# matheusfalcaopinto/triple-hybrid-rag

Hardware: AMD Instinct MI355X
Metric: queries/sec (fused top-10) (higher is better)
Workload: dtype f16 MFMA shortlist scan (f32 accumulate) + f64 rescoring of the f32 rows

## Files before the change

### triple-hybrid-rag_amd/csrc/dense.hip

```cpp
#include <stdlib.h>

#include "dense_common.hpp"

namespace thr {

constexpr double QREG_AIM_1M = 1448.0;
constexpr int QREG_KS = 32;
struct DenseKnobs {
    bool forced_q;
    int shape;
    bool forced32;
    double aim_1m;
    int ks;
};
static const DenseKnobs& dense_knobs() {
    static const DenseKnobs knobs = [] {
        DenseKnobs K;
        const char* e = getenv("THR_DENSE_F16");
        K.forced_q = e && e[0] == 'q';
        e = getenv("THR_DENSE_MFMA");
        K.shape = (e && atoi(e) == 32) ? 32 : 16;
        e = getenv("THR_DENSE_QW");
        K.forced32 = e && atoi(e) == 32;
        e = getenv("THR_DENSE_AIM");
        K.aim_1m = (e && atof(e) >= 64.0) ? atof(e) : QREG_AIM_1M;
        e = getenv("THR_DENSE_KS");
        K.ks = (e && atoi(e) >= 4 && atoi(e) <= 64) ? atoi(e) : QREG_KS;
        return K;
    }();
    return knobs;
}

bool qreg_staggered(int dim) { return !dense_knobs().forced_q && dim <= 768; }
int qreg_waves(int dim) { return qreg_staggered(dim) ? 8 : 4; }
int qreg_shape(int) { return dense_knobs().shape; }
int qreg_qw(int dim) {
    return (dim == 1024 && !qreg_staggered(dim) && qreg_shape(dim) == 16 && !dense_knobs().forced32) ? 48 : 32;
}
int qreg_max_queries(int dim) {
    const int qt = qreg_qw(dim) * qreg_waves(dim);
    const int64_t m = (int64_t)UINT32_MAX / ((int64_t)CAND_CAP * (int64_t)sizeof(Cand));
    return (int)(m / qt * qt);
}


static thread_local int f16_selected = THR_DENSE_F16_BY_DIM;
static bool f16_tuned_dim(int dim) { return dim == 512 || dim == 768 || dim == 1024; }
static bool f16_dim_ok(int dim, bool packed) { return f16_tuned_dim(dim) || (!packed && anydim_ok(dim)); }
static bool f16_anydim(int dim, bool packed) {
    return !packed && anydim_ok(dim) && (!f16_tuned_dim(dim) || f16_selected == THR_DENSE_F16_ANYDIM);
}

static DensePlan make_plan(void* ws, int64_t n_docs, int n_queries, int kprime, int kind, int dim,
                           bool packed) {
    DensePlan p;
    p.kind = kind;
    p.packed = kind == KIND_F16 && packed;
    p.anydim = kind == KIND_F16 && f16_anydim(dim, p.packed);
    p.nq = (kind == KIND_F16 && !p.packed && !p.anydim) ? f16_pick_nq(dim) : 1;
    p.row_bits = (kind == KIND_F16 && !p.packed) ? ROW_BITS_F16 : ROW_BITS;
    p.qtile = p.packed ? qreg_qw(dim) * qreg_waves(dim)
              : p.anydim ? anydim_qt(dim)
              : kind == KIND_F16 ? 32 * p.nq : MF_QT;
    p.ntiles = (n_queries + p.qtile - 1) / p.qtile;
    p.qpad = p.ntiles * p.qtile;
    const int64_t groups = (n_docs + MF_ROWS - 1) / MF_ROWS;
    p.sampled = n_docs > CAND_CAP / 2;
    const int ks_cap = p.packed ? dense_knobs().ks : 64;
    p.ksample = kprime < ks_cap ? kprime : ks_cap;
    double aim = (p.packed ? dense_knobs().aim_1m : 4096.0) * sqrt((double)n_docs / 1.0e6);
    const double aim_lo = 8.0 * kprime < 4096.0 ? 8.0 * kprime : 4096.0;
    aim = aim < aim_lo ? aim_lo : aim > 4096.0 ? 4096.0 : aim;
    int64_t target = (int64_t)((double)n_docs * (double)p.ksample / aim);
    if (target > SAMPLE_MAX) target = SAMPLE_MAX;
    if (target < 4 * (int64_t)p.ksample) target = 4 * (int64_t)p.ksample;
    int64_t sg = (target + MF_ROWS - 1) / MF_ROWS;
    if (sg > groups) sg = groups;
    p.sample_stride = sg > 0 ? groups / sg : 1;
    if (p.sample_stride < 1) p.sample_stride = 1;
    p.sample_groups = p.sampled ? sg : 0;
    p.sample_docs = p.sample_groups * MF_ROWS;
    p.groups = groups;
    p.tile_cap = p.packed ? 1 : p.qtile * (CAND_CAP / 2);
    const size_t qpad = (size_t)p.qpad;
    Arena A{(char*)ws};
    p.tau = A.take<float>(qpad);
    p.qerr = A.take<float>(qpad);
    if (kind != KIND_F16) p.qerr = nullptr;
    p.cnt = A.take<int>(qpad * (p.packed ? QREG_MAX_SEG : 1));
    p.tcnt = A.take<int>(p.ntiles);
    p.cand = A.take<Cand>(qpad * CAND_CAP);
    p.tlist = A.take<Cand>((size_t)p.ntiles * p.tile_cap);
    p.sample = A.take<float>(p.packed ? qpad * (size_t)QREG_MAX_SEG * SAMPLE_TOP : qpad * (size_t)p.sample_docs);
    p.qfrag = A.take<_Float16>(p.packed ? qpad * (size_t)dim : 0);
    p.sel_rows = A.take<int32_t>(qpad * SEL_BIG_BAND);
    p.sel_meta = A.take<int32_t>(4 * qpad);
    p.total = A.total;
    return p;
}

dim3 scan_grid(int ntiles, int64_t n_row_tiles, int waves, bool* shared_rows, int blocks_per_cu,
               int m_cap) {
    const int cus = num_cus() * blocks_per_cu;
    int64_t m_max = n_row_tiles / (8 * (int64_t)waves);
    if (m_max < 1) m_max = 1;
    if (m_max > m_cap) m_max = m_cap;
    int best_m = 1;
    double best_eff = 0.0;
    for (int m = 1; m <= (int)m_max; ++m) {
        const int64_t g = 8 * (int64_t)m * ntiles;
        const int64_t rounds = (g + cus - 1) / cus;
        const double eff = (double)g / (double)(rounds * cus);
        if (eff > best_eff + 1e-9) {
            best_eff = eff;
            best_m = m;
        }
    }
    *shared_rows = ntiles > 1;
    return dim3((unsigned)(8 * best_m * ntiles), 1u);
}

bool scan_nt(bool shared_rows) { return !shared_rows; }


template <int MODE>
static int launch_scan(const DensePlan& P, const DenseIndex& X, const DenseBatch& B, int* nseg = nullptr) {
    constexpr bool all = MODE == MODE_ALL;
    const int64_t units = all ? P.sample_groups : P.groups, stride = all ? P.sample_stride : 1;
    const float* tau = all ? nullptr : P.tau;
    float* smp = all ? P.sample : nullptr;
    const int64_t ld = all ? P.sample_docs : 0;
    if (P.packed)
        return launch_scan_f16q<MODE>(X.dim, X.docs16, P.qfrag, P.ntiles, units, stride, tau,
                                      all ? nullptr : P.cnt, all ? nullptr : P.cand, smp, B.st,
                                      nseg, X.doc_coll, B.query_coll, B.n_queries);
    const int32_t* doc_coll = all ? nullptr : X.doc_coll;
    const int32_t* query_coll = all ? nullptr : B.query_coll;
    int* tcnt = all ? nullptr : P.tcnt;
    Cand* tlist = all ? nullptr : P.tlist;
    const int tile_cap = all ? 0 : P.tile_cap;
    if (P.anydim)
        return launch_scan_anydim<MODE>(X.dim, X.docs, X.inv_norm, X.n_docs, B.queries, B.n_queries, P.ntiles,
                                        units, stride, tau, tcnt, tlist, tile_cap, smp, ld, B.st, doc_coll,
                                        query_coll);
    if (P.kind == KIND_F16)
        return launch_scan_f16<MODE>(X.dim, P.nq, X.docs, X.inv_norm, X.n_docs, B.queries, B.n_queries,
                                     P.ntiles, units, stride, tau, tcnt, tlist, tile_cap, smp, ld, B.st,
                                     doc_coll, query_coll);
    return launch_scan_mfma<MODE>(X.dim, X.docs, X.inv_norm, X.n_docs, B.queries, B.n_queries, P.ntiles,
                                  units, stride, tau, tcnt, tlist, tile_cap, smp, ld, B.st, doc_coll,
                                  query_coll);
}

static int dense_pipeline(const DensePlan& P, const DenseIndex& X, const DenseBatch& B,
                          const DensePhase& S) {
    int rc, nseg = 0, sample_nseg = 0;
    if (S.phase != PIPE_FINISH) {
        if (!P.packed) {
            hipError_t e = hipMemsetAsync(P.cnt, 0, (char*)P.cand - (char*)P.cnt, B.st);
            if (e != hipSuccess) return (int)e;
        }
        if (P.packed && (rc = launch_pack_queries(X.dim, B.queries, B.n_queries, P.qpad, P.qfrag, P.qerr, B.st)))
            return rc;
        if (P.sampled && (rc = launch_scan<MODE_ALL>(P, X, B, &sample_nseg))) return rc;
        if ((rc = launch_threshold(P, X, B, P.packed ? sample_nseg : 0))) return rc;
        if ((rc = launch_scan<MODE_FILTER>(P, X, B, &nseg))) return rc;
        if (!P.packed && (rc = launch_bucket(P, B.st))) return rc;
    } else if (P.packed) {
        if ((rc = launch_scan_f16q<MODE_FILTER, true>(X.dim, X.docs16, P.qfrag, P.ntiles, P.groups, 1,
                                                      nullptr, nullptr, nullptr, nullptr, B.st, &nseg)))
            return rc;
    }
    if ((rc = launch_band(P, X, B, S, nseg))) return rc;
    if (S.phase == PIPE_SHORTLIST) return THR_OK;
    return launch_rescore(P, X, B);
}

}

using namespace thr;

extern "C" size_t thr_dense_workspace_bytes(int64_t n_docs, int dim, int n_queries, int kprime) {
    if (n_docs <= 0 || n_queries <= 0) return 0;
    return make_plan(nullptr, n_docs, n_queries, kprime, KIND_F32, dim, false).total;
}

static int dense_args_ok(const void* docs, const void* dnorm, const void* inv_norm,
                         const void* queries, const void* a, const void* b, const void* c,
                         const void* d, const void* ws, int64_t n_docs, int n_queries, int k,
                         int kprime) {
    THR_RETURN_IF(!docs || !dnorm || !inv_norm || !queries || !a || !b || !c || !d || !ws,
                  THR_ERR_INVALID);
    THR_RETURN_IF(n_docs <= 0 || n_queries <= 0 || k <= 0 || kprime < k ||
                      kprime > THR_DENSE_MAX_K,
                  THR_ERR_INVALID);
    return THR_OK;
}

extern "C" int thr_dense_topk(const float* docs, const double* dnorm, const float* inv_norm,
                              int64_t n_docs, int dim, int64_t id_base, const float* queries,
                              int n_queries, int k, int kprime, const int32_t* doc_coll,
                              const int32_t* query_coll, double* out_scores,
                              int64_t* out_ids, int32_t* out_counts, uint32_t* out_flags,
                              void* workspace, size_t workspace_bytes, thr_stream_t stream) {
    clear_status();
    int rc = dense_args_ok(docs, dnorm, inv_norm, queries, out_scores, out_ids, out_counts,
                           out_flags, workspace, n_docs, n_queries, k, kprime);
    if (rc) return rc;
    THR_RETURN_IF((query_coll != nullptr) != (doc_coll != nullptr), THR_ERR_INVALID);
    THR_RETURN_IF(dim <= 0 || dim % CHUNK != 0 || dim / CHUNK > 4, THR_ERR_UNSUPPORTED);
    THR_RETURN_IF(n_docs >= (int64_t)1 << ROW_BITS, THR_ERR_UNSUPPORTED);
    const DensePlan P = make_plan(workspace, n_docs, n_queries, kprime, KIND_F32, dim, false);
    THR_RETURN_IF(workspace_bytes < P.total, THR_ERR_WORKSPACE);
    const DenseIndex X{docs, inv_norm, n_docs, dim, dnorm, id_base, doc_coll};
    const DenseBatch B{queries, n_queries, k, kprime, query_coll, (hipStream_t)stream,
                       out_scores, out_ids, out_counts, out_flags};
    return dense_pipeline(P, X, B, DensePhase{});
}

extern "C" size_t thr_dense_f16_workspace_bytes(int64_t n_docs, int dim, int n_queries,
                                                int kprime) {
    if (n_docs <= 0 || n_queries <= 0) return 0;
    const size_t a = make_plan(nullptr, n_docs, n_queries, kprime, KIND_F16, dim, false).total;
    if (anydim_ok(dim) && !f16_tuned_dim(dim)) return a;
    const size_t b = make_plan(nullptr, n_docs, n_queries, kprime, KIND_F16, dim, true).total;
    return a > b ? a : b;
}

extern "C" int thr_dense_f16_select(int flavour) {
    const int before = f16_selected;
    if (!f16_tiles_agree()) return before;
    if (flavour == THR_DENSE_F16_BY_DIM || flavour == THR_DENSE_F16_ANYDIM) f16_selected = flavour;
    return before;
}

extern "C" int thr_dense_f16_max_queries(int dim, int packed) {
    if (!f16_dim_ok(dim, packed != 0)) return 0;
    return packed ? qreg_max_queries(dim) : INT32_MAX;
}

extern "C" int thr_dense_f16_query_tile(int dim, int packed, int n_queries) {
    if (!f16_dim_ok(dim, packed != 0)) return 0;
    (void)n_queries;
    if (f16_anydim(dim, packed != 0)) return anydim_qt(dim);
    return packed ? qreg_qw(dim) * qreg_waves(dim) : 32 * f16_pick_nq(dim);
// ... 159 lines not shown
```

### triple-hybrid-rag_amd/csrc/dense_common.hpp

```cpp
#pragma once
#include <type_traits>

#include "thr_common.hpp"

namespace thr {

constexpr int CHUNK = 256;
constexpr int MODE_ALL = 0, MODE_FILTER = 1;
constexpr int CAND_CAP = 16384;
constexpr int SAMPLE_MAX = 1 << 20;
constexpr int WBUF = 256;
constexpr int ROW_BITS = 27;
constexpr uint32_t ROW_MASK = (1u << ROW_BITS) - 1;
constexpr int ROW_BITS_F16 = 25;
constexpr int SEL_BIG_BAND = 1024;
constexpr int QREG_MAX_SEG = 1024;
constexpr int SAMPLE_TOP = 4;
constexpr int CS_BINS = 4096;

struct Cand {
    float score;
    uint32_t doc;
};

// ... 42 lines not shown
    const half4 a = __builtin_convertvector(lo, half4), b = __builtin_convertvector(hi, half4);
    half8 v = {a[0], a[1], a[2], a[3], b[0], b[1], b[2], b[3]};
    return __builtin_bit_cast(f32x4, v);
}

inline size_t f16_lds_bytes(int dim, int nq) {
    return sizeof(_Float16) * 32 * nq * (size_t)dim +
           (sizeof(Cand) * WBUF + sizeof(float4) * MF2_STAGE_F4) * H_WAVES;
}
inline int f16_pick_nq(int dim) { return f16_lds_bytes(dim, 2) <= 160 * 1024 ? 2 : 1; }

inline bool anydim_ok(int dim) {
    return dim >= THR_DENSE_ANYDIM_STEP && dim <= THR_DENSE_ANYDIM_MAX && dim % THR_DENSE_ANYDIM_STEP == 0;
}
inline int anydim_qt(int dim) { return dim <= 768 ? 64 : dim <= 1536 ? 32 : 16; }
inline size_t anydim_lds_bytes(int dim) {
    return sizeof(_Float16) * (size_t)anydim_qt(dim) * (size_t)dim + sizeof(Cand) * WBUF * H_WAVES;
}

inline bool f16_tiles_agree() {
    for (int dim : {512, 768, 1024})
        if (anydim_qt(dim) != 32 * f16_pick_nq(dim)) return false;
    return true;
}

inline double scan_eps(int dim) {
    const double u = 5.9604644775390625e-08;
    return ((double)dim + 16.0) * u;
}

constexpr int KIND_F32 = 0, KIND_F16 = 1;
struct DensePlan {
    int kind;
    bool anydim;
    bool packed;
    int nq, qtile, ntiles, qpad, row_bits, ksample, tile_cap;
    bool sampled;
    int64_t groups, sample_groups, sample_stride, sample_docs;
    float* tau;
    float* qerr;
    int* cnt;
    int* tcnt;
    Cand *cand, *tlist;
    float* sample;
    _Float16* qfrag;
    int32_t *sel_rows, *sel_meta;
    size_t total;
};
struct DenseIndex {
    const float *docs, *inv_norm;
    int64_t n_docs;
    int dim;
    const double* dnorm = nullptr;
    int64_t id_base = 0;
    const int32_t* doc_coll = nullptr;
    const _Float16* docs16 = nullptr;
    double doc_rel_err = 0.0;
};
struct DenseBatch {
    const float* queries;
    int n_queries, k, kprime;
    const int32_t* query_coll;
    hipStream_t st;
    double* out_scores = nullptr;
    int64_t* out_ids = nullptr;
    int32_t* out_counts = nullptr;
    uint32_t* out_flags = nullptr;
};
enum { PIPE_ALL = 0, PIPE_SHORTLIST = 1, PIPE_FINISH = 2 };
struct DensePhase {
    int phase = PIPE_ALL;
    float* top_lb = nullptr;
    int top_m = 0;
    const float* gfloor = nullptr;
    const float* lb_all = nullptr;
    int n_shards = 0;
};

bool qreg_staggered(int dim);
int qreg_waves(int dim);
int qreg_shape(int dim);
int qreg_qw(int dim);
int qreg_max_queries(int dim);
dim3 scan_grid(int ntiles, int64_t n_row_tiles, int waves, bool* shared_rows, int blocks_per_cu = 1,
               int m_cap = 64);
bool scan_nt(bool shared_rows);

template <int MODE>
int launch_scan_mfma(int dim, const float* docs, const float* inv_norm, int64_t n_docs,
                     const float* queries, int n_queries, int ntiles, int64_t n_row_tiles,
                     int64_t tile_stride, const float* tau, int* tile_cnt, Cand* tile_list,
                     int tile_cap, float* sample, int64_t sample_ld, hipStream_t st,
                     const int32_t* doc_coll = nullptr, const int32_t* query_coll = nullptr);
template <int MODE>
int launch_scan_f16(int dim, int nq, const float* rows32, const float* inv_norm, int64_t n_docs,
                    const float* queries, int n_queries, int ntiles, int64_t n_row_tiles,
                    int64_t tile_stride, const float* tau, int* tile_cnt, Cand* tile_list,
                    int tile_cap, float* sample, int64_t sample_ld, hipStream_t st,
                    const int32_t* doc_coll = nullptr, const int32_t* query_coll = nullptr);
template <int MODE>
int launch_scan_anydim(int dim, const float* rows32, const float* inv_norm, int64_t n_docs,
                       const float* queries, int n_queries, int ntiles, int64_t n_row_tiles,
                       int64_t tile_stride, const float* tau, int* tile_cnt, Cand* tile_list,
                       int tile_cap, float* sample, int64_t sample_ld, hipStream_t st,
                       const int32_t* doc_coll = nullptr, const int32_t* query_coll = nullptr);
template <int MODE, bool PROF = false>
int launch_scan_f16q(int dim, const _Float16* rows16, const _Float16* qfrag, int n_qtiles,
                     int64_t n_row_tiles, int64_t tile_stride, const float* tau, int* seg_cnt,
                     Cand* cand, float* sample, hipStream_t st,
                     int* nseg_out = nullptr, const int32_t* doc_coll = nullptr,
                     const int32_t* query_coll = nullptr, int n_queries = 1 << 30,
                     unsigned long long* stamps = nullptr, int* n_blocks = nullptr);
int launch_pack_queries(int dim, const float* queries, int n_queries, int qpad, _Float16* qfrag,
                        float* qerr, hipStream_t st);
int launch_quantize_f16(const float* docs, int64_t n_docs, int dim, _Float16* docs16,
                        unsigned int* max_rel_err, hipStream_t st);
int launch_threshold(const DensePlan& P, const DenseIndex& X, const DenseBatch& B, int sample_nseg);
int launch_bucket(const DensePlan& P, hipStream_t st);
int launch_band(const DensePlan& P, const DenseIndex& X, const DenseBatch& B, const DensePhase& S, int nseg);
int launch_rescore(const DensePlan& P, const DenseIndex& X, const DenseBatch& B);
int launch_merge_scoped(const double* slab_s, const int64_t* slab_id, int n_queries, int n_slabs, int k,
                        int64_t id_base, const int32_t* query_scope, int n_scopes, double* out_scores,
                        int64_t* out_ids, int32_t* out_counts, uint32_t* out_flags, hipStream_t st);

}
```

### triple-hybrid-rag_amd/csrc/dense_scan_f16q.hip

```cpp
#include "dense_scan_f16q.hpp"

namespace thr {

template <int MODE, bool PROF>
int launch_scan_f16q(int dim, const _Float16* rows16, const _Float16* qfrag, int n_qtiles,
                            int64_t n_row_tiles, int64_t tile_stride, const float* tau, int* seg_cnt,
                            Cand* cand, float* sample, hipStream_t st,
                            int* nseg_out, const int32_t* doc_coll,
                            const int32_t* query_coll, int n_queries,
                            unsigned long long* stamps, int* n_blocks) {
    bool shared_rows = false;
    const bool stag = qreg_staggered(dim);
    const dim3 grid = scan_grid(n_qtiles, n_row_tiles, 1, &shared_rows, (!stag && dim <= 768) ? 2 : 1, 32);
    const int shape = qreg_shape(dim);
    const int nseg = (shape == 16 ? 4 : 2) * (int)(grid.x / n_qtiles);
    if (nseg_out) *nseg_out = nseg;
    if (n_blocks) *n_blocks = (int)grid.x;
    if (PROF && !stamps) return THR_OK;
#define THR_QS_LAUNCH(DIM, SHAPE)                                                                 \
    return launch_lds(dense_scan_f16qs<DIM, MODE, SHAPE>, grid, dim3(QS_NW * 64),                 \
                      QStag<DIM>::LDS_BYTES, st, (const f32x4*)rows16, (const f32x4*)qfrag,       \
                      n_qtiles, n_row_tiles, tile_stride, tau, seg_cnt, cand, CAND_CAP / nseg,    \
                      sample, doc_coll, query_coll, n_queries);
    if (stag) {
        if (dim == 512 && shape == 32) THR_QS_LAUNCH(512, 32)
        if (dim == 512) THR_QS_LAUNCH(512, 16)
        if (shape == 32) THR_QS_LAUNCH(768, 32)
        THR_QS_LAUNCH(768, 16)
    }
#undef THR_QS_LAUNCH
#define THR_Q_LAUNCH(DIM, SHAPE)                                                                  \
    return launch_lds(dense_scan_f16q<DIM, MODE, PROF, SHAPE>, grid, dim3(Q_NW * 64),             \
                      QScan<DIM>::LDS_BYTES, st, (const f32x4*)rows16, (const f32x4*)qfrag,       \
                      n_qtiles, n_row_tiles, tile_stride, tau, seg_cnt, cand, CAND_CAP / nseg,    \
                      sample, doc_coll, query_coll, n_queries, stamps);
    switch (dim) {
        case 512: if (shape == 16) THR_Q_LAUNCH(512, 16) THR_Q_LAUNCH(512, 32)
        case 768: if (shape == 16) THR_Q_LAUNCH(768, 16) THR_Q_LAUNCH(768, 32)
        case 1024:
            if (shape == 16 && qreg_qw(dim) == 48) THR_Q_LAUNCH(1024, 48)
            if (shape == 16) THR_Q_LAUNCH(1024, 16)
            THR_Q_LAUNCH(1024, 32)
        default: return THR_ERR_UNSUPPORTED;
    }
#undef THR_Q_LAUNCH
}

int launch_pack_queries(int dim, const float* queries, int n_queries, int qpad,
                               _Float16* qfrag, float* qerr, hipStream_t st) {
    const dim3 grid((unsigned)(qpad / 32));
    const bool s16 = qreg_shape(dim) == 16;
#define THR_PACK(DIM, SHAPE) \
    hipLaunchKernelGGL((pack_queries_f16<DIM, SHAPE>), grid, dim3(256), 0, st, queries, n_queries, (f32x4*)qfrag, qerr)
    switch (dim) {
        case 512: if (s16) THR_PACK(512, 16); else THR_PACK(512, 32); break;
        case 768: if (s16) THR_PACK(768, 16); else THR_PACK(768, 32); break;
        case 1024: if (s16) THR_PACK(1024, 16); else THR_PACK(1024, 32); break;
        default: return THR_ERR_UNSUPPORTED;
    }
#undef THR_PACK
    return launch_status();
}

int launch_quantize_f16(const float* docs, int64_t n_docs, int dim, _Float16* docs16,
                        unsigned int* max_rel_err, hipStream_t st) {
    if (docs16) {
        THR_RETURN_IF(dim % 16 != 0, THR_ERR_UNSUPPORTED);
        const int64_t n_pad = (n_docs + 31) / 32 * 32;
        hipLaunchKernelGGL(quantize_f16_norm, dim3((unsigned)((n_pad + 3) / 4)), dim3(256), 0, st,
                           docs, n_docs, dim, qreg_shape(dim), docs16, max_rel_err);
        return launch_status();
    }
    hipLaunchKernelGGL(measure_f16_error, dim3((unsigned)((n_docs + 3) / 4)), dim3(256), 0, st, docs,
                       n_docs, dim, max_rel_err);
    return launch_status();
}

#define THR_INSTANTIATE(MODE, PROF)                                                                    \
    template int launch_scan_f16q<MODE, PROF>(int, const _Float16*, const _Float16*, int, int64_t, int64_t, \
                                              const float*, int*, Cand*, float*, hipStream_t, int*, \
                                              const int32_t*, const int32_t*, int, unsigned long long*, int*);
THR_INSTANTIATE(MODE_ALL, false)
THR_INSTANTIATE(MODE_FILTER, false)
THR_INSTANTIATE(MODE_FILTER, true)
#undef THR_INSTANTIATE

}
```

### triple-hybrid-rag_amd/csrc/dense_scan_f16q.hpp

```cpp
#pragma once
#include "dense_common.hpp"

namespace thr {

constexpr int Q_RING = 4;
constexpr int Q_NW = 4;

template <int DIM>
struct QScan {
    static constexpr int KS = DIM / 16;
    static constexpr int HS = KS / 2;
    static constexpr int HALF_BYTES = HS * 1024;
    static constexpr int PER_CU = DIM <= 768 ? 2 : 1;
    static constexpr int NB = (160 * 1024 / PER_CU) / HALF_BYTES > 4 ? 4 : (160 * 1024 / PER_CU) / HALF_BYTES;
    static constexpr int PER = HS / Q_NW;
#ifndef THR_Q_RING_1024
#define THR_Q_RING_1024 8
#endif
    static constexpr int RING = PER_CU == 1 ? THR_Q_RING_1024 : Q_RING;
#ifdef Q_PROBE_EXTRA
    static constexpr int VM_PER_PIECE = 2, LDS_BYTES = NB * HALF_BYTES + 32 * 1024;
#else
    static constexpr int VM_PER_PIECE = 1, LDS_BYTES = NB * HALF_BYTES;
#endif
    static_assert(HS % Q_NW == 0 && NB >= 3, "half tile must split evenly over the waves; >= 3 buffers");
};

template <int DIM, int SHAPE>
__global__ __launch_bounds__(256) void pack_queries_f16(const float* __restrict__ queries,
                                                        int n_queries, f32x4* __restrict__ qfrag,
                                                        float* __restrict__ qerr) {
    constexpr int KS = DIM / 16;
    const int lane = threadIdx.x & 63, wave = threadIdx.x >> 6;
    __shared__ double red[4][4][32];
    double e = 0.0, nn = 0.0, e_hi = 0.0, n_hi = 0.0;
#pragma unroll 4
    for (int s = wave; s < KS; s += 4) {
        int q, d0;
        if constexpr (SHAPE == 32) {
            q = blockIdx.x * 32 + (lane & 31);
            d0 = 16 * s + 8 * (lane >> 5);
        } else {
            q = blockIdx.x * 32 + 16 * (s / (KS / 2)) + (lane & 15);
            d0 = 32 * (s % (KS / 2)) + 8 * (lane >> 4);
        }
        f32x4 lo = {0.f, 0.f, 0.f, 0.f}, hi = lo;
        if (q < n_queries) {
            const f32x4* src = reinterpret_cast<const f32x4*>(queries + (int64_t)q * DIM + d0);
            lo = src[0];
            hi = src[1];
        }
        const f32x4 packed = pack_f16x8(lo, hi);
        qfrag[((int64_t)blockIdx.x * KS + s) * 64 + lane] = packed;
        const half8 hv = __builtin_bit_cast(half8, packed);
        double e1 = 0.0, n1 = 0.0;
#pragma unroll
        for (int j = 0; j < 8; ++j) {
            const float v = j < 4 ? lo[j] : hi[j - 4];
            const double d = (double)v - (double)(float)hv[j];
            e1 += d * d;
            n1 += (double)v * (double)v;
        }
        if (SHAPE == 32 || s < KS / 2) {
            e += e1;
            nn += n1;
        } else {
            e_hi += e1;
            n_hi += n1;
        }
    }
    if constexpr (SHAPE == 32) {
        e += __shfl_xor(e, 32, WAVE);
        nn += __shfl_xor(nn, 32, WAVE);
        if (lane < 32) {
            red[wave][0][lane] = e;
            red[wave][1][lane] = nn;
        }
    } else {
#pragma unroll
        for (int m = 16; m <= 32; m <<= 1) {
            e += __shfl_xor(e, m, WAVE);
            nn += __shfl_xor(nn, m, WAVE);
            e_hi += __shfl_xor(e_hi, m, WAVE);
            n_hi += __shfl_xor(n_hi, m, WAVE);
        }
        if (lane < 16) {
            red[wave][0][lane] = e;
            red[wave][1][lane] = nn;
            red[wave][0][16 + lane] = e_hi;
            red[wave][1][16 + lane] = n_hi;
        }
    }
    __syncthreads();
    if (threadIdx.x < 32) {
        double es = 0.0, ns = 0.0;
#pragma unroll
        for (int w = 0; w < 4; ++w) {
            es += red[w][0][threadIdx.x];
            ns += red[w][1][threadIdx.x];
        }
        const float rel = ns > 0.0 ? (float)sqrt(es / ns) : 0.f;
        qerr[blockIdx.x * 32 + threadIdx.x] = __uint_as_float(__float_as_uint(rel) + 1u);
    }
}

#define QS_RD(dst, ks) \
    asm volatile("ds_read_b128 %0, %1 offset:%2" : "=v"(dst) : "v"(abase), "n"((ks) * 1024) : "memory")
template <int S, int HS, int RING>
__device__ __forceinline__ void qs_fill(f32x4 (&a)[RING], uint32_t abase) {
    if constexpr (S < RING && S < HS) {
        QS_RD(a[S], S);
        qs_fill<S + 1, HS>(a, abase);
    }
}
template <int SHAPE>
struct QAcc;
template <>
struct QAcc<32> {
    static constexpr int NQL = 1, SEGS = 2;
    static constexpr int QW = 32, NQB = 2, NREG = 16;
    f32x16 v;
    __device__ __forceinline__ void zero() {
#pragma unroll
        for (int x = 0; x < 16; ++x) v[x] = 0.f;
    }
    template <int X> __device__ __forceinline__ float get() const { return v[X]; }
    template <int X> static __device__ __forceinline__ int row(int lane) { return (X & 3) + 8 * (X >> 2) + 4 * (lane >> 5); }
    template <int X> static constexpr int qsel() { return 0; }
    static __device__ __forceinline__ int query(int lane, int) { return lane & 31; }
    static __device__ __forceinline__ int seg(int lane) { return lane >> 5; }
};
template <>
struct QAcc<48> {
    static constexpr int NQL = 3, SEGS = 4;
    static constexpr int QW = 48, NQB = 3, NREG = 24;
    f32x4 t[6];
    __device__ __forceinline__ void zero() {
#pragma unroll
        for (int x = 0; x < 6; ++x) t[x] = f32x4{0.f, 0.f, 0.f, 0.f};
    }
    template <int X> __device__ __forceinline__ float get() const { return t[X >> 2][X & 3]; }
    template <int X> static __device__ __forceinline__ int row(int lane) { return 16 * ((X >> 2) / 3) + 4 * (lane >> 4) + (X & 3); }
    template <int X> static constexpr int qsel() { return (X >> 2) % 3; }
    static __device__ __forceinline__ int query(int lane, int qb) { return 16 * qb + (lane & 15); }
    static __device__ __forceinline__ int seg(int lane) { return lane >> 4; }
};
template <>
struct QAcc<16> {
    static constexpr int NQL = 2, SEGS = 4;
    static constexpr int QW = 32, NQB = 2, NREG = 16;
    f32x4 t[4];
    __device__ __forceinline__ void zero() {
#pragma unroll
        for (int x = 0; x < 4; ++x) t[x] = f32x4{0.f, 0.f, 0.f, 0.f};
    }
    template <int X> __device__ __forceinline__ float get() const { return t[X >> 2][X & 3]; }
    template <int X> static __device__ __forceinline__ int row(int lane) { return 16 * (X >> 3) + 4 * (lane >> 4) + (X & 3); }
    template <int X> static constexpr int qsel() { return (X >> 2) & 1; }
    static __device__ __forceinline__ int query(int lane, int qb) { return 16 * qb + (lane & 15); }
    static __device__ __forceinline__ int seg(int lane) { return lane >> 4; }
};

template <int S, int K0, int KS, int SHAPE, int NBQ>
__device__ __forceinline__ void qsx_mfma(const f32x4& a, const f32x4 (&bq)[NBQ], QAcc<SHAPE>& acc) {
    if constexpr (SHAPE == 32) {
        acc.v = __builtin_amdgcn_mfma_f32_32x32x16_f16(__builtin_bit_cast(half8, a),
                                                       __builtin_bit_cast(half8, bq[K0 + S]), acc.v, 0, 0, 0);
    } else {
        constexpr int k32 = (K0 + S) / 2, ra = S & 1, NQB = QAcc<SHAPE>::NQB;
        static_assert(NBQ == NQB * KS / 2, "one B fragment per 16-query block and 32-dim step");
        static_for<0, NQB>([&](auto qb) {
            acc.t[NQB * ra + qb] = __builtin_amdgcn_mfma_f32_16x16x32_f16(
                __builtin_bit_cast(half8, a), __builtin_bit_cast(half8, bq[qb * (KS / 2) + k32]),
                acc.t[NQB * ra + qb], 0, 0, 0);
        });
    }
}
template <int S, int HS, int K0, int KS, int PER, int SHAPE, int RING, int NBQ, typename Issue>
__device__ __forceinline__ void qsx_steps(f32x4 (&a)[RING], const f32x4 (&bq)[NBQ], QAcc<SHAPE>& acc,
                                          uint32_t abase, Issue& issue_piece) {
    if constexpr (S < HS) {
        constexpr int left = HS - S - 1 < RING - 1 ? HS - S - 1 : RING - 1;
        asm volatile("s_waitcnt lgkmcnt(%1)" : "+v"(a[S % RING]) : "n"(left) : "memory");
        qsx_mfma<S, K0, KS, SHAPE>(a[S % RING], bq, acc);
        if constexpr (S + RING < HS) QS_RD(a[S % RING], S + RING);
// ... 581 lines not shown
```

### triple-hybrid-rag_amd/csrc/dense_select.hip

```cpp
#include "dense_common.hpp"

namespace thr {

constexpr int BUCKET_BLOCKS = 32;
__global__ __launch_bounds__(256) void bucket_candidates(const int* __restrict__ tile_cnt,
                                                         const Cand* __restrict__ tile_list,
                                                         int tile_cap, int qtile, int row_bits,
                                                         int* __restrict__ cand_cnt,
                                                         Cand* __restrict__ cand) {
    __shared__ int count[128], base[128], fill[128];
    const uint32_t row_mask = (1u << row_bits) - 1u;
    const int tile = blockIdx.y;
    int n = tile_cnt[tile];
    n = n < tile_cap ? n : tile_cap;
    const int per = (n + gridDim.x - 1) / gridDim.x;
    const int lo = blockIdx.x * per, hi = lo + per < n ? lo + per : n;
    const Cand* list = tile_list + (int64_t)tile * tile_cap;
    if (threadIdx.x < 128) count[threadIdx.x] = fill[threadIdx.x] = 0;
    __syncthreads();
    for (int i = lo + threadIdx.x; i < hi; i += blockDim.x)
        atomicAdd(&count[list[i].doc >> row_bits], 1);
    __syncthreads();
    if (threadIdx.x < qtile && count[threadIdx.x] > 0)
        base[threadIdx.x] = atomicAdd(&cand_cnt[tile * qtile + threadIdx.x], count[threadIdx.x]);
// ... 148 lines not shown
                nn += (double)v * (double)v;
            }
        red[0][threadIdx.x] = e;
        red[1][threadIdx.x] = nn;
        __syncthreads();
        for (int o = 128; o > 0; o >>= 1) {
            if (threadIdx.x < o) {
                red[0][threadIdx.x] += red[0][threadIdx.x + o];
                red[1][threadIdx.x] += red[1][threadIdx.x + o];
            }
            __syncthreads();
        }
        if (threadIdx.x == 0) {
            float rel = red[1][0] > 0.0 ? (float)sqrt(red[0][0] / red[1][0]) : 0.f;
            qerr[q] = __uint_as_float(__float_as_uint(rel) + 1u);
        }
    }
    if (query_is_void(queries, n_queries, dim, q, &flag)) {
        if (threadIdx.x == 0) tau[q] = INFINITY;
        return;
    }
    if (n_sample < kk) {
        if (threadIdx.x == 0) tau[q] = -INFINITY;
        return;
    }
    const float* s = sample_scores + (int64_t)q * sample_ld;
    const int qc = (query_coll && q < n_queries) ? query_coll[q] : -1;
    auto val = [&](int i) {
        float v = s[i];
        if (qc != -1) {
            const int64_t row = (int64_t)(i / unit) * stride * unit + i % unit;
            if (row >= n_docs || doc_coll[row] != qc) v = -INFINITY;
        }
        return v;
    };
    __shared__ float kred[4];
    __shared__ int kcnt;
    const int lane = threadIdx.x & 63, wave = threadIdx.x >> 6;
    auto sweep = [&](auto&& fn) {
        for (int base = threadIdx.x; base < n_sample; base += 8 * 256) {
            float v[8];
#pragma unroll
            for (int u = 0; u < 8; ++u) v[u] = base + u * 256 < n_sample ? val(base + u * 256) : -INFINITY;
#pragma unroll
            for (int u = 0; u < 8; ++u) fn(v[u]);
        }
    };
    float m = -INFINITY;
    sweep([&](float v) { m = fmaxf(m, v); });
#pragma unroll
    for (int o = 32; o > 0; o >>= 1) m = fmaxf(m, __shfl_xor(m, o, WAVE));
    if (lane == 0) kred[wave] = m;
    if (threadIdx.x == 0) kcnt = 0;
    for (int i = threadIdx.x; i < CS_BINS; i += 256) hist[i] = 0;
    __syncthreads();
    m = fmaxf(fmaxf(kred[0], kred[1]), fmaxf(kred[2], kred[3]));
    if (m > 0.f && m < INFINITY) {
        const float thr = 0.5f * m, scale = 4095.f / (m - thr);
        int c = 0;
        sweep([&](float v) {
            if (v >= thr) {
                const int bn = (int)((v - thr) * scale);
                atomicAdd(&hist[bn > CS_BINS - 1 ? CS_BINS - 1 : bn], 1);
                ++c;
            }
        });
#pragma unroll
        for (int o = 32; o > 0; o >>= 1) c += __shfl_xor(c, o, WAVE);
        if (lane == 0 && c) atomicAdd(&kcnt, c);
        __syncthreads();
        if (kcnt >= kk) {
            coarse_find_bin(hist, kk, aux);
            if (threadIdx.x == 0) tau[q] = thr + (float)aux[0] / scale;
            return;
        }
        __syncthreads();
    }
    const uint32_t key = block_coarse_select([&](int i) { return fkey(val(i)); }, n_sample, kk, hist, aux);
    if (threadIdx.x == 0) tau[q] = coarse_value(key);
}

constexpr int KT_REG = 16;
static_assert(QREG_MAX_SEG * SAMPLE_TOP <= 256 * KT_REG, "kth_select_top holds every kept value in registers");
__global__ __launch_bounds__(256) void kth_select_top(const float* __restrict__ sample, int n_vals, int kk,
                                                      const float* __restrict__ queries, int n_queries,
                                                      int dim, float* __restrict__ tau) {
    __shared__ int hist[256];
    __shared__ int wsum[4];
    __shared__ int bc[2];
    __shared__ int flag;
    const int q = blockIdx.x, t = threadIdx.x, lane = t & 63, wave = t >> 6;
    if (query_is_void(queries, n_queries, dim, q, &flag)) {
        if (t == 0) tau[q] = INFINITY;
        return;
    }
    if (n_vals < kk) {
        if (t == 0) tau[q] = -INFINITY;
        return;
    }
    uint32_t key[KT_REG];
#pragma unroll
    for (int u = 0; u < KT_REG; ++u) {
        const int i = t + u * 256;
        key[u] = fkey(i < n_vals ? sample[(int64_t)q * n_vals + i] : -INFINITY);
    }
    uint32_t prefix = 0, mask = 0;
    int remaining = kk;
#pragma unroll 1
    for (int shift = 24; shift >= 0; shift -= 8) {
        hist[t] = 0;
        __syncthreads();
#pragma unroll
        for (int u = 0; u < KT_REG; ++u)
            if (t + u * 256 < n_vals && (key[u] & mask) == prefix) atomicAdd(&hist[(key[u] >> shift) & 255], 1);
        __syncthreads();
        const int mine = hist[255 - t];
        int incl = mine;
#pragma unroll
        for (int o = 1; o < 64; o <<= 1) {
            const int v = __shfl_up(incl, o, WAVE);
            if (lane >= o) incl += v;
        }
        if (lane == 63) wsum[wave] = incl;
        __syncthreads();
        for (int x = 0; x < wave; ++x) incl += wsum[x];
        if (incl - mine < remaining && remaining <= incl) {
            bc[0] = 255 - t;
            bc[1] = incl - mine;
        }
        __syncthreads();
        remaining -= bc[1];
        prefix |= (uint32_t)bc[0] << shift;
        mask |= 255u << shift;
    }
    if (t == 0) tau[q] = fkey_inv(prefix);
}

constexpr int SEL_THREADS = 256;
constexpr int SEL_REG = 16;
constexpr int SEL_FLAT = 8192;
static size_t band_lds_bytes(int dim) { return sizeof(float) * dim + sizeof(int) * CS_BINS; }
constexpr int CAPB = SEL_BIG_BAND;
template <bool TOPM>
__global__ __launch_bounds__(SEL_THREADS, 4) void select_band(
    int dim, const float* __restrict__ queries, const float* __restrict__ tau,
    const int* __restrict__ cand_cnt, const Cand* __restrict__ cand,
    const int* __restrict__ tile_cnt, int tile_cap, int qtile, int k, int kprime, double eps32,
    double doc_relerr, const float* __restrict__ qerr, int nseg, int seg_cap,
    const int32_t* __restrict__ doc_coll, const int32_t* __restrict__ query_coll,
    int32_t* __restrict__ sel_rows, int32_t* __restrict__ sel_meta,
    const float* __restrict__ gfloor, const float* __restrict__ lb_all, int n_shards, int lb_m,
    float* __restrict__ top_lb, int top_m) {
    extern __shared__ float4 lds_sel[];
    __shared__ int aux[8];
    __shared__ int bc[4];
    __shared__ int32_t s_id[CAPB];
    __shared__ int n_sel;
    __shared__ double wsum[4];
    float* lds_qv = reinterpret_cast<float*>(lds_sel);
    int* hist = reinterpret_cast<int*>(lds_sel + dim / 4);

    const int q = blockIdx.x;
    const int lane = threadIdx.x & 63, wave = threadIdx.x >> 6;
    const double eq = qerr ? (double)qerr[q] : 0.0;
    const double eps = eps32 + doc_relerr * (1.0 + eq) + eq;
    const Cand* c = cand + (int64_t)q * CAND_CAP;
// ... 230 lines not shown
        __syncthreads();
        for (int u = 0; u < my_n; ++u) {
            const Cand e = load_cand(u);
            if (fkey(e.score) == tkey) {
                const int p = atomicAdd(&n_sel, 1);
                if (p < top_m) o[p] = lowered(e.score);
            }
        }
        return;
    }
    if (band_lo > -INFINITY) {
#pragma unroll
        for (int u = 0; u < SEL_REG; ++u) {
            const bool in = u < my_n && mine[u].score >= band_lo;
            const unsigned long long m = __ballot(in);
            if (m) {
                int base = 0;
                if (lane == 0) base = atomicAdd(&n_sel, __popcll(m));
                base = __shfl(base, 0, WAVE);
                const int p = base + __popcll(m & ((1ull << lane) - 1ull));
                if (in && p < CAPB) s_id[p] = mine[u].doc;
            }
        }
        for (int u = SEL_REG; u < my_n; ++u) {
            const Cand e = load_cand(u);
            if (e.score >= band_lo) {
                const int p = atomicAdd(&n_sel, 1);
                if (p < CAPB) s_id[p] = e.doc;
            }
        }
        __syncthreads();
        if (n_sel <= CAPB) {
            floor32 = fmaxf(floor32, band_lo);
            band_done = true;
        } else {
            __syncthreads();
            if (threadIdx.x == 0) n_sel = 0;
            __syncthreads();
        }
    }
    if (!band_done) {
        if (n > kprime) {
            const uint32_t tkey = block_radix_select_local(
                [&](int u) { return fkey(load_cand(u).score); }, my_n, kprime, hist, bc);
            floor32 = fkey_inv(tkey);
            for (int u = 0; u < my_n; ++u) {
                const Cand e = load_cand(u);
                if (fkey(e.score) > tkey) {
                    const int p = atomicAdd(&n_sel, 1);
                    s_id[p] = e.doc;
                }
            }
            __syncthreads();
            for (int u = 0; u < my_n; ++u) {
                const Cand e = load_cand(u);
                if (fkey(e.score) == tkey) {
                    const int p = atomicAdd(&n_sel, 1);
                    if (p < kprime) s_id[p] = e.doc;
                }
            }
            __syncthreads();
            if (threadIdx.x == 0 && n_sel > kprime) n_sel = kprime;
        } else {
            for (int u = 0; u < my_n; ++u) {
                const Cand e = load_cand(u);
                if (e.score > -INFINITY) {
                    const int p = atomicAdd(&n_sel, 1);
                    s_id[p] = e.doc;
                }
            }
        }
    }
    __syncthreads();
    const int ns = n_sel;
    for (int i = threadIdx.x; i < ns; i += SEL_THREADS) sel_rows[(int64_t)q * CAPB + i] = s_id[i];
    if (threadIdx.x == 0) {
        sel_meta[4 * q + 0] = ns;
        sel_meta[4 * q + 1] = (int32_t)__float_as_uint(floor32);
        sel_meta[4 * q + 2] = overflow ? 1 : 0;
        sel_meta[4 * q + 3] = (int32_t)__float_as_uint(gF);
    }
}

__global__ __launch_bounds__(256) void dense_floor_kernel(const float* __restrict__ lb, int n_shards,
                                                          int n_queries, int m, int k,
                                                          float* __restrict__ gfloor) {
    extern __shared__ float fl_v[];
    const int q = blockIdx.x, n = n_shards * m;
    for (int i = threadIdx.x; i < n; i += blockDim.x)
        fl_v[i] = lb[((int64_t)(i / m) * n_queries + q) * m + i % m];
    if (threadIdx.x == 0) gfloor[q] = -INFINITY;
    __syncthreads();
    if (n < k) return;
    for (int i = threadIdx.x; i < n; i += blockDim.x) {
        const float v = fl_v[i];
        if (!(v > -INFINITY)) continue;
        int rank = 0;
        for (int j = 0; j < n; ++j) {
            const float w = fl_v[j];
            rank += (w > v || (w == v && j < i)) ? 1 : 0;
        }
        if (rank == k - 1) gfloor[q] = v;
    }
}

int launch_threshold(const DensePlan& P, const DenseIndex& X, const DenseBatch& B, int sample_nseg) {
    if (P.sampled && sample_nseg > 0) {
        hipLaunchKernelGGL(kth_select_top, dim3(P.qpad), dim3(256), 0, B.st, (const float*)P.sample,
                           sample_nseg * SAMPLE_TOP, P.ksample, B.queries, B.n_queries, X.dim, P.tau);
        return launch_status();
    }
    hipLaunchKernelGGL(kth_select, dim3(P.qpad), dim3(256), 0, B.st,
                       P.sampled ? (const float*)P.sample : nullptr, P.sample_docs, (int)P.sample_docs,
                       P.ksample, B.queries, B.n_queries, X.dim, P.tau, P.packed ? nullptr : P.qerr,
                       X.doc_coll, B.query_coll, MF_ROWS, P.sampled ? P.sample_stride : (int64_t)1,
                       X.n_docs);
    return launch_status();
}

int launch_bucket(const DensePlan& P, hipStream_t st) {
    hipLaunchKernelGGL(bucket_candidates, dim3(BUCKET_BLOCKS, P.ntiles), dim3(256), 0, st, P.tcnt,
                       P.tlist, P.tile_cap, P.qtile, P.row_bits, P.cnt, P.cand);
    return launch_status();
}

int launch_band(const DensePlan& P, const DenseIndex& X, const DenseBatch& B, const DensePhase& S,
                int nseg) {
    const bool topm = S.phase == PIPE_SHORTLIST;
    hipLaunchKernelGGL(topm ? select_band<true> : select_band<false>, dim3(B.n_queries),
                       dim3(SEL_THREADS), band_lds_bytes(X.dim), B.st, X.dim, B.queries, P.tau, P.cnt,
                       P.cand, P.tcnt, P.tile_cap, P.qtile, B.k, B.kprime, scan_eps(X.dim),
                       X.doc_rel_err, P.qerr, nseg, nseg ? CAND_CAP / nseg : 0, X.doc_coll,
                       B.query_coll, P.sel_rows, P.sel_meta, S.gfloor, S.lb_all, S.n_shards,
                       topm ? 0 : S.top_m, S.top_lb, topm ? S.top_m : 0);
    return launch_status();
}

}

using namespace thr;

extern "C" int thr_dense_floor(const float* top_lb, int n_shards, int n_queries, int m, int k,
                               float* gfloor, thr_stream_t stream) {
    clear_status();
    THR_RETURN_IF(!top_lb || !gfloor || n_shards <= 0 || n_queries <= 0 || m <= 0 || k <= 0, THR_ERR_INVALID);
    THR_RETURN_IF((int64_t)n_shards * m > 8192, THR_ERR_CAPACITY);
    hipLaunchKernelGGL(dense_floor_kernel, dim3(n_queries), dim3(256), sizeof(float) * n_shards * m,
                       (hipStream_t)stream, top_lb, n_shards, n_queries, m, k, gfloor);
    return launch_status();
}
```

Baseline: 780,800.

## Select sampled kth threshold with one wave per query via ballot bisection

Adds a wave-per-query threshold kernel that keeps the sampled top values in registers and finds the kth key by 32-step bitwise bisection using ballot/popcount, in place of a 256-thread block-per-query histogram select. The void-query check moves into the pack kernel, which now pre-writes tau as +inf for empty queries and -inf otherwise, so the select kernel no longer rereads the query vectors. The aim is a cheaper threshold stage with less block-level synchronisation, at the cost of more registers per lane for large sample counts. The old block path stays reachable through an environment variable.

```diff
diff --git a/triple-hybrid-rag_amd/csrc/dense.hip b/triple-hybrid-rag_amd/csrc/dense.hip
--- a/triple-hybrid-rag_amd/csrc/dense.hip
+++ b/triple-hybrid-rag_amd/csrc/dense.hip
@@ -1,4 +1,5 @@
 #include <stdlib.h>
+#include <string.h>
 
 #include "dense_common.hpp"
 
@@ -12,6 +13,7 @@
     bool forced32;
     double aim_1m;
     int ks;
+    bool select_block;
 };
 static const DenseKnobs& dense_knobs() {
     static const DenseKnobs knobs = [] {
@@ -26,11 +28,14 @@
         K.aim_1m = (e && atof(e) >= 64.0) ? atof(e) : QREG_AIM_1M;
         e = getenv("THR_DENSE_KS");
         K.ks = (e && atoi(e) >= 4 && atoi(e) <= 64) ? atoi(e) : QREG_KS;
+        e = getenv("THR_DENSE_SELECT");
+        K.select_block = e && strcmp(e, "block") == 0;
         return K;
     }();
     return knobs;
 }
 
+bool dense_select_block() { return dense_knobs().select_block; }
 bool qreg_staggered(int dim) { return !dense_knobs().forced_q && dim <= 768; }
 int qreg_waves(int dim) { return qreg_staggered(dim) ? 8 : 4; }
 int qreg_shape(int) { return dense_knobs().shape; }
@@ -160,7 +165,7 @@
             hipError_t e = hipMemsetAsync(P.cnt, 0, (char*)P.cand - (char*)P.cnt, B.st);
             if (e != hipSuccess) return (int)e;
         }
-        if (P.packed && (rc = launch_pack_queries(X.dim, B.queries, B.n_queries, P.qpad, P.qfrag, P.qerr, B.st)))
+        if (P.packed && (rc = launch_pack_queries(X.dim, B.queries, B.n_queries, P.qpad, P.qfrag, P.qerr, P.tau, B.st)))
             return rc;
         if (P.sampled && (rc = launch_scan<MODE_ALL>(P, X, B, &sample_nseg))) return rc;
         if ((rc = launch_threshold(P, X, B, P.packed ? sample_nseg : 0))) return rc;
diff --git a/triple-hybrid-rag_amd/csrc/dense_common.hpp b/triple-hybrid-rag_amd/csrc/dense_common.hpp
--- a/triple-hybrid-rag_amd/csrc/dense_common.hpp
+++ b/triple-hybrid-rag_amd/csrc/dense_common.hpp
@@ -148,6 +148,7 @@
 int qreg_shape(int dim);
 int qreg_qw(int dim);
 int qreg_max_queries(int dim);
+bool dense_select_block();
 dim3 scan_grid(int ntiles, int64_t n_row_tiles, int waves, bool* shared_rows, int blocks_per_cu = 1,
                int m_cap = 64);
 bool scan_nt(bool shared_rows);
@@ -178,7 +179,7 @@
                      const int32_t* query_coll = nullptr, int n_queries = 1 << 30,
                      unsigned long long* stamps = nullptr, int* n_blocks = nullptr);
 int launch_pack_queries(int dim, const float* queries, int n_queries, int qpad, _Float16* qfrag,
-                        float* qerr, hipStream_t st);
+                        float* qerr, float* tau, hipStream_t st);
 int launch_quantize_f16(const float* docs, int64_t n_docs, int dim, _Float16* docs16,
                         unsigned int* max_rel_err, hipStream_t st);
 int launch_threshold(const DensePlan& P, const DenseIndex& X, const DenseBatch& B, int sample_nseg);
diff --git a/triple-hybrid-rag_amd/csrc/dense_scan_f16q.hip b/triple-hybrid-rag_amd/csrc/dense_scan_f16q.hip
--- a/triple-hybrid-rag_amd/csrc/dense_scan_f16q.hip
+++ b/triple-hybrid-rag_amd/csrc/dense_scan_f16q.hip
@@ -47,11 +47,11 @@
 }
 
 int launch_pack_queries(int dim, const float* queries, int n_queries, int qpad,
-                               _Float16* qfrag, float* qerr, hipStream_t st) {
+                               _Float16* qfrag, float* qerr, float* tau, hipStream_t st) {
     const dim3 grid((unsigned)(qpad / 32));
     const bool s16 = qreg_shape(dim) == 16;
 #define THR_PACK(DIM, SHAPE) \
-    hipLaunchKernelGGL((pack_queries_f16<DIM, SHAPE>), grid, dim3(256), 0, st, queries, n_queries, (f32x4*)qfrag, qerr)
+    hipLaunchKernelGGL((pack_queries_f16<DIM, SHAPE>), grid, dim3(256), 0, st, queries, n_queries, (f32x4*)qfrag, qerr, tau)
     switch (dim) {
         case 512: if (s16) THR_PACK(512, 16); else THR_PACK(512, 32); break;
         case 768: if (s16) THR_PACK(768, 16); else THR_PACK(768, 32); break;
diff --git a/triple-hybrid-rag_amd/csrc/dense_scan_f16q.hpp b/triple-hybrid-rag_amd/csrc/dense_scan_f16q.hpp
--- a/triple-hybrid-rag_amd/csrc/dense_scan_f16q.hpp
+++ b/triple-hybrid-rag_amd/csrc/dense_scan_f16q.hpp
@@ -29,7 +29,8 @@
 template <int DIM, int SHAPE>
 __global__ __launch_bounds__(256) void pack_queries_f16(const float* __restrict__ queries,
                                                         int n_queries, f32x4* __restrict__ qfrag,
-                                                        float* __restrict__ qerr) {
+                                                        float* __restrict__ qerr,
+                                                        float* __restrict__ tau) {
     constexpr int KS = DIM / 16;
     const int lane = threadIdx.x & 63, wave = threadIdx.x >> 6;
     __shared__ double red[4][4][32];
@@ -101,6 +102,7 @@
         }
         const float rel = ns > 0.0 ? (float)sqrt(es / ns) : 0.f;
         qerr[blockIdx.x * 32 + threadIdx.x] = __uint_as_float(__float_as_uint(rel) + 1u);
+        if (tau) tau[blockIdx.x * 32 + threadIdx.x] = ns == 0.0 ? INFINITY : -INFINITY;
     }
 }
 
diff --git a/triple-hybrid-rag_amd/csrc/dense_select.hip b/triple-hybrid-rag_amd/csrc/dense_select.hip
--- a/triple-hybrid-rag_amd/csrc/dense_select.hip
+++ b/triple-hybrid-rag_amd/csrc/dense_select.hip
@@ -254,6 +254,7 @@
 
 constexpr int KT_REG = 16;
 static_assert(QREG_MAX_SEG * SAMPLE_TOP <= 256 * KT_REG, "kth_select_top holds every kept value in registers");
+static_assert(QREG_MAX_SEG * SAMPLE_TOP <= 64 * 64, "kth_select_top_wave: at most 64 kept values per lane");
 __global__ __launch_bounds__(256) void kth_select_top(const float* __restrict__ sample, int n_vals, int kk,
                                                       const float* __restrict__ queries, int n_queries,
                                                       int dim, float* __restrict__ tau) {
@@ -650,6 +651,47 @@
     }
 }
 
+constexpr int SW_WAVES = 4;
+template <typename CountGe>
+__device__ __forceinline__ uint32_t wave_select_key(CountGe count_ge, int kk) {
+    uint32_t t = 0;
+#pragma unroll 1
+    for (int bit = 31; bit >= 0; --bit) {
+        const uint32_t c = t | (1u << bit);
+        if (count_ge(c) >= kk) t = c;
+    }
+    return t;
+}
+
+template <int R>
+__global__ __launch_bounds__(64 * SW_WAVES) void kth_select_top_wave(const float* __restrict__ sample,
+                                                                     int n_vals, int kk, int qpad,
+                                                                     float* __restrict__ tau) {
+    const int lane = threadIdx.x & 63;
+    const int q = blockIdx.x * SW_WAVES + (int)(threadIdx.x >> 6);
+    if (q >= qpad) return;
+    if (tau[q] == INFINITY) return;
+    if (n_vals < kk) {
+        if (lane == 0) tau[q] = -INFINITY;
+        return;
+    }
+    uint32_t key[R];
+#pragma unroll
+    for (int u = 0; u < R; ++u) {
+        const int i = lane + u * 64;
+        key[u] = i < n_vals ? fkey(sample[(int64_t)q * n_vals + i]) : 0u;
+    }
+    const uint32_t t = wave_select_key(
+        [&](uint32_t c) {
+            int m = 0;
+#pragma unroll
+            for (int u = 0; u < R; ++u) m += __popcll(__ballot(key[u] >= c));
+            return m;
+        },
+        kk);
+    if (lane == 0) tau[q] = fkey_inv(t);
+}
+
 __global__ __launch_bounds__(256) void dense_floor_kernel(const float* __restrict__ lb, int n_shards,
                                                           int n_queries, int m, int k,
                                                           float* __restrict__ gfloor) {
@@ -673,6 +715,18 @@
 }
 
 int launch_threshold(const DensePlan& P, const DenseIndex& X, const DenseBatch& B, int sample_nseg) {
+    if (P.sampled && sample_nseg > 0 && !dense_select_block()) {
+        const int n_vals = sample_nseg * SAMPLE_TOP;
+        const dim3 grid((unsigned)((P.qpad + SW_WAVES - 1) / SW_WAVES)), block(64 * SW_WAVES);
+#define THR_KTW(R) \
+    hipLaunchKernelGGL(kth_select_top_wave<R>, grid, block, 0, B.st, (const float*)P.sample, n_vals, P.ksample, P.qpad, P.tau)
+        if (n_vals <= 512) THR_KTW(8);
+        else if (n_vals <= 1024) THR_KTW(16);
+        else if (n_vals <= 2048) THR_KTW(32);
+        else THR_KTW(64);
+#undef THR_KTW
+        return launch_status();
+    }
     if (P.sampled && sample_nseg > 0) {
         hipLaunchKernelGGL(kth_select_top, dim3(P.qpad), dim3(256), 0, B.st, (const float*)P.sample,
                            sample_nseg * SAMPLE_TOP, P.ksample, B.queries, B.n_queries, X.dim, P.tau);
```

After: 777,100. About the same (-0.5%).
